# z430/keyword-spotting

Measured on AMD Instinct MI355X. Metric: 1s 16kHz clips/sec end-to-end (wav->label), higher is better.
Workload: dtype f32

## Files before the change

keyword-spotting_amd/csrc/kws_dscnn.hip:

```cpp
#include <array>
#include <utility>

#include "kws_dscnn_stages.h"

namespace kws {
namespace {

#ifndef KWS_X_DSCNN_STAMP_TID
#define KWS_X_DSCNN_STAMP_TID 0
#endif

__device__ __forceinline__ DscnnWeights weights_for_this_clip() {
#if defined(__HIP_DEVICE_COMPILE__)
    using KArg = const __attribute__((address_space(4))) DscnnWeights*;
    KArg p = (KArg)__builtin_amdgcn_kernarg_segment_ptr();
    asm volatile("" : "+s"(p));
    return *p;
#else
    return DscnnWeights{};
#endif
}

using FwdKernelFn = void (*)(DscnnWeights, const float*, int, float*, int32_t*, float*, unsigned long long*, const int*, StreamPush);
struct FwdKernelArgs {
    DscnnWeights w;
    const float* feat;
    int B;
    float* logits;
    int32_t* label;
    float* act;
    unsigned long long* stamps;
    const int* ring_hops;
    StreamPush sp;
};

__device__ __forceinline__ ScanWindows scan_windows_now() {
#if defined(__HIP_DEVICE_COMPILE__)
    using KArg = const __attribute__((address_space(4))) FwdKernelArgs*;
    KArg p = (KArg)__builtin_amdgcn_kernarg_segment_ptr();
    asm volatile("" : "+s"(p));
    return p->sp.scan;
#else
    return ScanWindows{};
#endif
}

template <bool SCAN>
__device__ __forceinline__ const float* clip_features(const float* __restrict__ feat, int clip, const ScanWindows& sw) {
    if constexpr (SCAN) {
        unsigned rec = __umulhi((unsigned)clip, sw.wpr_recip), win = (unsigned)clip - rec * sw.wpr;
        if (win >= sw.wpr) {
            win -= sw.wpr;
            ++rec;
        }
        return feat + (size_t)rec * sw.row_floats + (size_t)win * sw.win_floats;
    } else {
        return feat + (size_t)clip * (IN_T * IN_F);
    }
}

template <bool PAIR, bool SCAN = false>
__device__ __forceinline__ void stage_features_persist(float* lds, const float* __restrict__ feat, int clip, int tid,
                                                       const ScanWindows& sw = ScanWindows{}) {
    constexpr int ST = STAGE_WAVES * 64;
    constexpr int FV = (IN_T * IN_F + ST - 1) / ST;
    static_assert(2 * STAGE_WAVES == NW, "each staging wavefront zeroes the maximum slot of one other wavefront");
    const int lane = tid & 63, wv = tid >> 6;
    const float* f = clip_features<SCAN>(feat, clip, sw);
    float fv[FV];
#pragma unroll
    for (int k = 0; k < FV; ++k) {
        const int i = tid + k * ST;
        fv[k] = i < IN_T * IN_F ? f[i] : 0.f;
    }
    float* featp = lds + OFF_FEAT_P;
    for (int i = tid; i < FEAT_H * FEAT_W; i += ST) {
        const int r = i / FEAT_W - 2, c = i % FEAT_W - 2;
        if (!((unsigned)r < (unsigned)IN_T && (unsigned)c < (unsigned)IN_F)) featp[i] = 0.f;
    }
#pragma unroll
    for (int k = 0; k < FV; ++k) {
        const int i = tid + k * ST;
        if (i < IN_T * IN_F) featp[(i / IN_F + 2) * FEAT_W + (i % IN_F) + 2] = fv[k];
    }
    if constexpr (PAIR) {
        float m = 0.f;
#pragma unroll
        for (int k = 0; k < FV; ++k) m = fmaxf(m, fabsf(fv[k]));
        publish_wave_max(lds, 0, wv, lane, m);
        if (lane == 63) lds[OFF_WMAX + wv + STAGE_WAVES] = 0.f;
    }
}

__device__ __forceinline__ void pool_fc_wave(const DscnnWeights& w, const float* lds, int lane, int clip, float* __restrict__ logits,
                                             int32_t* __restrict__ label, float* __restrict__ a_pool) {
    const int C = w.num_classes;
    float4 fcw[CH / 4];
    float fcb = 0.f;
    const float4* wr = reinterpret_cast<const float4*>(w.fc_w + (lane < C ? lane : 0) * CH);
#pragma unroll
    for (int c = 0; c < CH / 4; ++c) fcw[c] = wr[c];
    if (lane < C) fcb = w.fc_b[lane];
    const float ring_b = w.pw_b[3 * CH + lane];
    constexpr float RING_N = 55.f * 11.f - 53.f * 9.f;
    float s = 0.f;
#pragma unroll
    for (int k = 0; k < NW; ++k) s += lds[OFF_POOLBUF_P + k * CH + lane];
    s = fmaf(RING_N, relu(ring_b), s) * (1.0f / (55.f * 11.f));
    if (a_pool) a_pool[lane] = s;
    float acc = fcb;
#pragma unroll
    for (int c = 0; c < CH / 4; ++c) {
        const float4 a4 = fcw[c];
        acc = fmaf(a4.x, __builtin_bit_cast(float, __builtin_amdgcn_readlane(__builtin_bit_cast(int, s), 4 * c + 0)), acc);
        acc = fmaf(a4.y, __builtin_bit_cast(float, __builtin_amdgcn_readlane(__builtin_bit_cast(int, s), 4 * c + 1)), acc);
        acc = fmaf(a4.z, __builtin_bit_cast(float, __builtin_amdgcn_readlane(__builtin_bit_cast(int, s), 4 * c + 2)), acc);
        acc = fmaf(a4.w, __builtin_bit_cast(float, __builtin_amdgcn_readlane(__builtin_bit_cast(int, s), 4 * c + 3)), acc);
    }
    if (lane < C) logits[(size_t)clip * C + lane] = acc;
    const int idx = wave_argmax_first(lane < C ? acc : -INFINITY, lane, C);
    if (label && lane == 0) label[clip] = idx;
}

template <int MODE, bool DIAG = true, bool PRECONV = false, bool STREAM = false, bool CLUSTER = false, bool PERSIST = false,
          bool SCAN = false>
__global__ __launch_bounds__(NT) void kws_dscnn_fwd_kernel(DscnnWeights w_arg, const float* __restrict__ feat, int B,
                                                           float* __restrict__ logits, int32_t* __restrict__ label,
                                                           float* __restrict__ act_arg,
                                                           unsigned long long* __restrict__ stamps_arg,
                                                           const int* __restrict__ ring_hops, StreamPush sp) {
    static_assert(!STREAM || (MODE >= 4 && !DIAG && !PRECONV), "the fused push exists for the product paths only");
    static_assert(!PERSIST || ((MODE == 4 || MODE == 5) && !PRECONV && !STREAM), "persistent workgroups: batched product paths only");
    static_assert(!SCAN || ((MODE == 4 || MODE == 5) && !DIAG && !PRECONV && !STREAM && !CLUSTER), "strided windows: batched product paths only");
    constexpr bool PAIR = MODE == 5;
    constexpr int NP = PAIR ? 2 : 3;
    BlockTables t1_pre{};
    static_assert(!CLUSTER || STREAM, "time-tile clusters exist for the streaming push only");
    float* const act = DIAG ? act_arg : nullptr;
    unsigned long long* const stamps = DIAG ? stamps_arg : nullptr;
    extern __shared__ __attribute__((aligned(16))) float lds[];
    constexpr bool MFMA = MODE != 0;
    const int tid_k = threadIdx.x;
    const int lane_k = tid_k & 63, wv_k = tid_k >> 6;

    const int cl_n = CLUSTER ? sp.cluster : 1;
    int clip = CLUSTER ? (int)blockIdx.x / cl_n : (int)blockIdx.x;
    const int cl_tile = CLUSTER ? (int)blockIdx.x - clip * cl_n : 0;
    if (clip >= B) return;
    const int j0 = Blk<4>::H * cl_tile / cl_n, j1 = Blk<4>::H * (cl_tile + 1) / cl_n;
    auto rows = [&](int lo, int hi, int H, int W) { return PosRange{(lo < 0 ? 0 : lo) * W, (hi > H ? H : hi) * W}; };
    const PosRange rg4 = rows(j0, j1, Blk<4>::H, Blk<4>::W), rg3 = rows(j0 - 2, j1, Blk<3>::H, Blk<3>::W),
                   rg2 = rows(j0 - 4, j1, Blk<2>::H, Blk<2>::W), rg1 = rows(j0 - 6, j1, Blk<1>::H, Blk<1>::W),
                   rg0 = rows(j0 - 7, j1 + 1, C1_H, C1_W);
    int n_stamp = 0;
    auto stamp = [&]() {
        if (stamps && tid_k == KWS_X_DSCNN_STAMP_TID) stamps[(size_t)clip * KWS_DSCNN_STAMPS + n_stamp] = __builtin_amdgcn_s_memtime();
        ++n_stamp;
    };

    constexpr bool SPLIT = MODE >= 4;
    BlockTables t1p{};
    uintx4 c1p[PERSIST ? 7 : 1][NP];
    int prev_clip = -1;
    float* a_prev = nullptr;
    if constexpr (PERSIST) {
        fetch_block_tables(w_arg, 1, tid_k, t1p);
        if (wv_k < STAGE_WAVES) stage_features_persist<PAIR, SCAN>(lds, feat, clip, tid_k, sp.scan);
        load_conv1_frags(w_arg, wv_k, lane_k, c1p);
        __syncthreads();
    }
    for (;;) {
    const DscnnWeights w = PERSIST ? weights_for_this_clip() : w_arg;
    int tid = tid_k;
    if constexpr (PERSIST) {
        int wv_l = __builtin_amdgcn_readfirstlane(wv_k), lane_l = lane_k;
        asm volatile("" : "+s"(wv_l), "+v"(lane_l));
        tid = (wv_l << 6) | (lane_l & 63);
    }
    const int lane = tid & 63, wv = tid >> 6;
    if constexpr (PERSIST) n_stamp = 0;
    if (stamps && tid == KWS_X_DSCNN_STAMP_TID) stamps[(size_t)clip * KWS_DSCNN_STAMPS + KWS_DSCNN_STAMPS - 2] = __builtin_amdgcn_s_memrealtime();
    stamp();

    PwOperands<MODE> wa;
    int hops_before = 0;
    int kx = 0, ky[5] = {0, 0, 0, 0, 0}, sg[5] = {0, 0, 0, 0, 0};
    if constexpr (PERSIST) {
        if constexpr (PAIR) {
            const float mxf = read_stage_max(lds, 0, 1);
            kx = pow2_exp_for(mxf);
            const float bz0 = (w.c1_abs * mxf + w.c1_bmax) * 1.001f;
            cap_units(kx, sg[0], w.k_c1, bz0);
            const float by1 = (w.dw_abs[0] * bz0 + w.dw_bmax[0]) * 1.001f;
            ky[1] = pow2_exp_for(by1);
            cap_units(ky[1], sg[1], w.k_pw[0], (w.pw_abs[0] * by1 + w.pw_bmax[0]) * 1.001f);
            store_block_tables(lds, 1, tid, t1p, pow2f(ky[1]), pow2f(sg[1]), pow2f(ky[1] - sg[0]));
            conv1_build_windows(lds, tid, pow2f(kx), OFF_FEAT_P);
            __syncthreads();
        } else {
            store_block_tables(lds, 1, tid, t1p);
        }
        stamp();
        conv1_phase_split<false, NP>(w, lds, tid, c1p, rg0, pow2f(kx), pow2f(sg[0]), OFF_FEAT_P);
        if (wv == NW - 1 && prev_clip >= 0) {
            pool_fc_wave(w, lds, lane, prev_clip, logits, label, a_prev);
            if (stamps && lane == 0) stamps[(size_t)prev_clip * KWS_DSCNN_STAMPS + 13] = __builtin_amdgcn_s_memtime();
        }
        load_afrag(w, 1, wv >= 4 ? wv - 4 : 0, lane, wa.ring[0]);
    } else if constexpr (PRECONV) {
        static_assert(!PRECONV || MODE >= 4, "the pre-convolved entry exists for the product (split) path only");
        const float* z = feat + (size_t)clip * (CH * P0);
        fetch_block_tables(w, 1, tid, t1_pre);
        float zmax = 0.f;
        for (int i = tid; i < CH * P0; i += NT) {
            const float v = z[i];
            lds[OFF_Z0 + pidx(i / P0, i % P0, P0 + 2)] = v;
            zmax = fmaxf(zmax, v);
        }
        if (tid < CH) {
            lds[OFF_Z0 + pidx(tid, P0, P0 + 2)] = 0.f;
            lds[OFF_Z0 + pidx(tid, P0 + 1, P0 + 2)] = 0.f;
        }
        if constexpr (PAIR)
            publish_wave_max(lds, 1, wv, lane, zmax);
        else
            store_block_tables(lds, 1, tid, t1_pre);
        if constexpr (Leftover<1>::HAS && (MODE == 4 || MODE == 5) && !CLUSTER)
            load_afrag(w, 1, wv >= 4 ? wv - 4 : 0, lane, wa.ring[0]);
        else
            load_block_head(w, 1, lane, wa);
        stamp();
    } else {
    float* featp = lds + OFF_FEAT;
    const float* f = clip_features<SCAN>(feat, clip, sp.scan);
    constexpr int FV = (IN_T * IN_F + NT - 1) / NT;
    float fv[FV];
    int row_new = -1;
    int head;
    if constexpr (STREAM) {
        hops_before = *sp.hops;
        const int K = (sp.p.frame_len + sp.p.frame_step - 1) / sp.p.frame_step;
        head = (((hops_before + 2 - K) % IN_T) + IN_T) % IN_T;
        const int step = sp.p.frame_step;
        const long f_start = (long)step * hops_before + step - (long)((sp.p.frame_len + step - 1) / step) * step;
        if (f_start >= 0) row_new = (int)((((f_start / step) - head) % IN_T + IN_T) % IN_T);
    } else {
        head = ring_hops ? (((*ring_hops + 1 - sp.frames_lag) % IN_T) + IN_T) % IN_T : 0;
    }
#pragma unroll
    for (int k = 0; k < FV; ++k) {
        const int i = tid + k * NT;
        fv[k] = (i < IN_T * IN_F && i / IN_F != row_new) ? f[((i / IN_F + head) % IN_T) * IN_F + i % IN_F] : 0.f;
    }
    BlockTables t1;
    fetch_block_tables(w, 1, tid, t1);
    __builtin_amdgcn_sched_barrier(0);
    float a1[SPLIT ? 1 : 50];
    uintx4 c1f[SPLIT ? 7 : 1][NP];
    if constexpr (SPLIT) {
        load_conv1_frags(w, wv, lane, c1f);
    } else if constexpr (MFMA) {
        const int half = lane >> 5, col = lane & 31, ct = wv & 1;
#pragma unroll
        for (int s = 0; s < 50; ++s) a1[s] = w.c1_w[(2 * s + half) * CH + ct * 32 + col];
        load_pointwise(w, 1, lane, wa);
    }
    __builtin_amdgcn_sched_barrier(0);
    if constexpr (PAIR) {
        float m = 0.f;
#pragma unroll
        for (int k = 0; k < FV; ++k) m = fmaxf(m, fabsf(fv[k]));
        publish_wave_max(lds, 0, wv, lane, m);
    }
    if constexpr (STREAM) {
#ifdef KWS_X_STREAM_NO_FRAME
        if (false)
#else
        if (wv == 0 && cl_tile == cl_n - 1)
#endif
            stream_frame_wave(sp.p, sp.t, sp.hop, clip, clip, false, sp.pcm_ring, sp.ring_len, const_cast<float*>(feat), hops_before,
                              reinterpret_cast<unsigned char*>(lds + OFF_Z2), lane,
                              row_new >= 0 ? featp + (row_new + 2) * FEAT_W + 2 : nullptr, sp.refine_ctr);
        for (int i = tid; i < FEAT_H * FEAT_W; i += NT) {
            const int r = i / FEAT_W - 2, c = i % FEAT_W - 2;
            if (!((unsigned)r < (unsigned)IN_T && (unsigned)c < (unsigned)IN_F)) featp[i] = 0.f;
        }
        if constexpr (!PAIR) store_block_tables(lds, 1, tid, t1);
#pragma unroll
        for (int k = 0; k < FV; ++k) {
            const int i = tid + k * NT;
            if (i < IN_T * IN_F && i / IN_F != row_new) featp[(i / IN_F + 2) * FEAT_W + (i % IN_F) + 2] = fv[k];
        }
        __syncthreads();
    } else {
    for (int i = tid; i < FEAT_H * FEAT_W; i += NT) {
        const int r = i / FEAT_W - 2, c = i % FEAT_W - 2;
        if (!((unsigned)r < (unsigned)IN_T && (unsigned)c < (unsigned)IN_F)) featp[i] = 0.f;
    }
    if constexpr (!PAIR) store_block_tables(lds, 1, tid, t1);
#pragma unroll
    for (int k = 0; k < FV; ++k) {
        const int i = tid + k * NT;
        if (i < IN_T * IN_F) featp[(i / IN_F + 2) * FEAT_W + (i % IN_F) + 2] = fv[k];
    }
    __syncthreads();
    }
    if constexpr (PAIR) {
        float mxf = read_stage_max(lds, 0, 1);
        if constexpr (STREAM) {
            if (row_new >= 0 && cl_tile == cl_n - 1)
                for (int c = 0; c < IN_F; ++c) mxf = fmaxf(mxf, fabsf(featp[(row_new + 2) * FEAT_W + 2 + c]));
        }
        kx = pow2_exp_for(mxf);
        const float bz0 = (w.c1_abs * mxf + w.c1_bmax) * 1.001f;
        cap_units(kx, sg[0], w.k_c1, bz0);
        const float by1 = (w.dw_abs[0] * bz0 + w.dw_bmax[0]) * 1.001f;
        ky[1] = pow2_exp_for(by1);
        cap_units(ky[1], sg[1], w.k_pw[0], (w.pw_abs[0] * by1 + w.pw_bmax[0]) * 1.001f);
        store_block_tables(lds, 1, tid, t1, pow2f(ky[1]), pow2f(sg[1]), pow2f(ky[1] - sg[0]));
        conv1_build_windows(lds, tid, pow2f(kx));
        __syncthreads();
    }
    stamp();

    if constexpr (SPLIT) {
        conv1_phase_split<CLUSTER, NP>(w, lds, tid, c1f, rg0, pow2f(kx), pow2f(sg[0]));
        if constexpr (Leftover<1>::HAS && (MODE == 4 || MODE == 5) && !CLUSTER)
            load_afrag(w, 1, wv >= 4 ? wv - 4 : 0, lane, wa.ring[0]);
        else
            load_block_head(w, 1, lane, wa);
    } else {
        conv1_phase<MFMA>(w, lds, tid, a1);
    }
    }
    stamp();
    __syncthreads();
    stamp();
    float* a = act ? act + (size_t)clip * KWS_ACT_FLOATS_PER_CLIP : nullptr;
    constexpr bool KSL_ON = (MODE == 4 || MODE == 5) && !CLUSTER;
    if (a) {
        const float u = PAIR ? pow2f(-sg[0]) : 1.f;
        for (int i = tid; i < CH * P0; i += NT) a[i] = lds[OFF_Z0 + pidx(i / P0, i % P0, P0 + 2)] * u;
        a += CH * P0;
    }
    PairCtx pc;
    if constexpr (PAIR && PRECONV) {
        const float mz0 = read_stage_max(lds, 1, 1);
        const float by1 = (w.dw_abs[0] * mz0 + w.dw_bmax[0]) * 1.001f;
        ky[1] = pow2_exp_for(by1);
        cap_units(ky[1], sg[1], w.k_pw[0], (w.pw_abs[0] * by1 + w.pw_bmax[0]) * 1.001f);
        store_block_tables(lds, 1, tid, t1_pre, pow2f(ky[1]), pow2f(sg[1]), pow2f(ky[1]));
        __syncthreads();
    }
    if constexpr (PAIR) {
        const float mz = read_stage_max(lds, 1, 1) * pow2f(-sg[0]);
        const float bz = (w.pw_abs[0] * ((w.dw_abs[0] * mz + w.dw_bmax[0]) * 1.001f) + w.pw_bmax[0]) * 1.001f;
        const float by = (w.dw_abs[1] * bz + w.dw_bmax[1]) * 1.001f;
        ky[2] = pow2_exp_for(by);
        cap_units(ky[2], sg[2], w.k_pw[1], (w.pw_abs[1] * by + w.pw_bmax[1]) * 1.001f);
        pc.s_dww = pow2f(ky[2] - sg[1]);
        pc.s_dwb = pow2f(ky[2]);
        pc.s_pwb = pow2f(sg[2]);
    }
    block_phase<1, MODE, CLUSTER>(w, lds, tid, wa, nullptr, rg1, pc);
    stamp();
    __syncthreads();
    if constexpr (Leftover<1>::HAS && KSL_ON) {
        leftover_combine<1, PAIR>(lds, tid);
        __syncthreads();
    }
    stamp();
    if (a) {
        const float u = PAIR ? pow2f(-sg[1]) : 1.f;
        for (int i = tid; i < CH * Blk<1>::POUT; i += NT)
            a[i] = lds[OFF_Z1 + pidx(i / Blk<1>::POUT, i % Blk<1>::POUT, Blk<1>::SOUT)] * u;
        a += CH * Blk<1>::POUT;
    }
    if constexpr (PAIR) {
        const float mz = fmaxf(read_stage_max(lds, 2, (Leftover<1>::HAS && KSL_ON) ? 2 : 1) * pow2f(-sg[1]), w.pw_bmax[0]);
        const float bz = (w.pw_abs[1] * ((w.dw_abs[1] * mz + w.dw_bmax[1]) * 1.001f) + w.pw_bmax[1]) * 1.001f;
        const float by = (w.dw_abs[2] * bz + w.dw_bmax[2]) * 1.001f;
        ky[3] = pow2_exp_for(by);
        cap_units(ky[3], sg[3], w.k_pw[2], (w.pw_abs[2] * by + w.pw_bmax[2]) * 1.001f);
        pc.s_dww = pow2f(ky[3] - sg[2]);
        pc.s_dwb = pow2f(ky[3]);
        pc.s_pwb = pow2f(sg[3]);
    }
    block_phase<2, MODE, CLUSTER>(w, lds, tid, wa, nullptr, rg2, pc);
    stamp();
    __syncthreads();
    if constexpr (Leftover<2>::HAS && KSL_ON) {
        leftover_combine<2, PAIR>(lds, tid);
        __syncthreads();
    }
    stamp();
    if (a) {
        const float u = PAIR ? pow2f(-sg[2]) : 1.f;
        for (int i = tid; i < CH * Blk<2>::POUT; i += NT)
            a[i] = lds[OFF_Z2 + pidx(i / Blk<2>::POUT, i % Blk<2>::POUT, Blk<2>::SOUT)] * u;
        a += CH * Blk<2>::POUT;
    }
    if constexpr (PAIR) {
        const float mz = fmaxf(read_stage_max(lds, 0, (Leftover<2>::HAS && KSL_ON) ? 2 : 1) * pow2f(-sg[2]), w.pw_bmax[1]);
        const float bz = (w.pw_abs[2] * ((w.dw_abs[2] * mz + w.dw_bmax[2]) * 1.001f) + w.pw_bmax[2]) * 1.001f;
        const float by = (w.dw_abs[3] * bz + w.dw_bmax[3]) * 1.001f;
        ky[4] = pow2_exp_for(by);
        cap_units(ky[4], sg[4], w.k_pw[3], (w.pw_abs[3] * by + w.pw_bmax[3]) * 1.001f);
        pc.s_dww = pow2f(ky[4] - sg[3]);
        pc.s_dwb = pow2f(ky[4]);
        pc.s_pwb = pow2f(sg[4]);
    }
    block_phase<3, MODE, CLUSTER>(w, lds, tid, wa, nullptr, rg3, pc);
    stamp();
    __syncthreads();
    stamp();
    if (a) {
        const float u = PAIR ? pow2f(-sg[3]) : 1.f;
        for (int i = tid; i < CH * Blk<3>::POUT; i += NT)
            a[i] = lds[OFF_Z3 + pidx(i / Blk<3>::POUT, i % Blk<3>::POUT, Blk<3>::SOUT)] * u;
        a += CH * Blk<3>::POUT;
    }
    if constexpr (PAIR) {
        pc.inv_out = pow2f(-sg[4]);
    }
    block_phase<4, MODE, CLUSTER>(w, lds, tid, wa, a ? a + CH : nullptr, rg4, pc,
                                  PERSIST ? OFF_POOLBUF_P : OFF_POOLBUF);
    stamp();
    if constexpr (PERSIST) {
        const int next = clip + (int)gridDim.x;
        __builtin_amdgcn_sched_barrier(0);
        const ScanWindows sw_next = SCAN ? scan_windows_now() : ScanWindows{};
        if (wv < STAGE_WAVES && next < B) stage_features_persist<PAIR, SCAN>(lds, feat, next, tid, sw_next);
        stamp();
        load_conv1_frags(w, wv, lane, c1p);
        __syncthreads();
        stamp();
        if (stamps && tid == KWS_X_DSCNN_STAMP_TID) stamps[(size_t)clip * KWS_DSCNN_STAMPS + KWS_DSCNN_STAMPS - 1] = __builtin_amdgcn_s_memrealtime();
        prev_clip = clip;
        a_prev = a;
        clip = next;
        if (clip >= B) break;
        continue;
    }
    const int C = w.num_classes;
    float4 fcw[CH / 4];
    float fcb = 0.f, ring_b = 0.f;
    if (wv == 0 && lane < C) {
        const float4* wr = reinterpret_cast<const float4*>(w.fc_w + lane * CH);
#pragma unroll
        for (int c = 0; c < CH / 4; ++c) fcw[c] = wr[c];
        fcb = w.fc_b[lane];
    }
    if (tid < CH) ring_b = w.pw_b[3 * CH + tid];
    __syncthreads();
    stamp();

    float* pooled = lds + OFF_POOLED;
    constexpr float RING_N = 55.f * 11.f - 53.f * 9.f;
    bool run_fc = true;
    if constexpr (CLUSTER) {
        float* part = sp.cl_part + ((size_t)clip * cl_n + cl_tile) * CH;
        if (tid < CH) {
            float s = 0.f;
#pragma unroll
            for (int k = 0; k < NW; ++k) s += lds[OFF_POOLBUF + k * CH + tid];
            __hip_atomic_store(part + tid, s, __ATOMIC_RELAXED, __HIP_MEMORY_SCOPE_AGENT);
        }
        asm volatile("s_waitcnt vmcnt(0)" ::: "memory");
        __syncthreads();
        int* last_flag = reinterpret_cast<int*>(lds + OFF_POOLED + CH);
        if (tid == 0) {
            const int arrived = atomicAdd(&sp.cl_count[clip], 1);
            *last_flag = arrived == cl_n - 1;
            if (arrived == cl_n - 1) sp.cl_count[clip] = 0;
        }
        __syncthreads();
        run_fc = *last_flag != 0;
        if (run_fc) {
            if (tid < CH) {
                float s = 0.f;
                for (int t = 0; t < cl_n; ++t)
                    s += __hip_atomic_load(sp.cl_part + ((size_t)clip * cl_n + t) * CH + tid, __ATOMIC_RELAXED, __HIP_MEMORY_SCOPE_AGENT);
                pooled[tid] = fmaf(RING_N, relu(ring_b), s) * (1.0f / (55.f * 11.f));
            }
        }
        __syncthreads();
    } else {
    if (tid < CH) {
        float s = 0.f;
#pragma unroll
        for (int k = 0; k < NW; ++k) s += lds[OFF_POOLBUF + k * CH + tid];
        s = fmaf(RING_N, relu(ring_b), s) * (1.0f / (55.f * 11.f));
        pooled[tid] = s;
        if (a) a[tid] = s;
    }
    __syncthreads();
    }

    if (run_fc && wv == 0) {
        float v = -INFINITY;
        if (lane < C) {
            float acc = fcb;
            const float4* pl = reinterpret_cast<const float4*>(pooled);
#pragma unroll
            for (int c = 0; c < CH / 4; ++c) {
                const float4 a4 = fcw[c], p4 = pl[c];
                acc = fmaf(a4.x, p4.x, acc);
                acc = fmaf(a4.y, p4.y, acc);
                acc = fmaf(a4.z, p4.z, acc);
                acc = fmaf(a4.w, p4.w, acc);
            }
            logits[(size_t)clip * C + lane] = acc;
            if constexpr (STREAM) {
                if (sp.h_logits) __hip_atomic_store(sp.h_logits + (size_t)clip * C + lane, acc, __ATOMIC_RELAXED, __HIP_MEMORY_SCOPE_SYSTEM);
            }
            v = acc;
        }
        const int idx = wave_argmax_first(v, lane, C);
        if (label && lane == 0) label[clip] = idx;
        if constexpr (STREAM) {
            if (sp.h_label && lane == 0) __hip_atomic_store(sp.h_label + clip, idx, __ATOMIC_RELAXED, __HIP_MEMORY_SCOPE_SYSTEM);
        }
    }
    if constexpr (STREAM) {
        int finishers = (int)gridDim.x;
        if constexpr (CLUSTER) finishers /= cl_n;
        if (sp.h_flag) asm volatile("s_waitcnt vmcnt(0)" ::: "memory");
        if (run_fc && tid == 0 && atomicAdd(&sp.hops[1], 1) == finishers - 1) {
            sp.hops[1] = 0;
            sp.hops[0] = hops_before + 1;
            if (sp.h_flag) __hip_atomic_store(sp.h_flag, hops_before + 1, __ATOMIC_RELAXED, __HIP_MEMORY_SCOPE_SYSTEM);
        }
    }
    stamp();
    if (stamps && tid == KWS_X_DSCNN_STAMP_TID) stamps[(size_t)clip * KWS_DSCNN_STAMPS + KWS_DSCNN_STAMPS - 1] = __builtin_amdgcn_s_memrealtime();
    break;
    }
    if constexpr (PERSIST) {
        if (wv_k == NW - 1) {
            pool_fc_wave(w_arg, lds, lane_k, prev_clip, logits, label, a_prev);
            if (stamps && lane_k == 0) stamps[(size_t)prev_clip * KWS_DSCNN_STAMPS + 13] = __builtin_amdgcn_s_memtime();
        }
    }
}

enum : unsigned { F_DIAG = 1, F_PRECONV = 2, F_STREAM = 4, F_CLUSTER = 8, F_PERSIST = 16, F_SCAN = 32 };
struct FwdVariant {
    int mode;
    unsigned flags;
    bool diag, preconv, stream, cluster, persist, scan;
    constexpr FwdVariant(int m, unsigned f)
        : mode(m), flags(f), diag(f & F_DIAG), preconv(f & F_PRECONV), stream(f & F_STREAM), cluster(f & F_CLUSTER), persist(f & F_PERSIST), scan(f & F_SCAN) {}
};
constexpr FwdVariant kFwdVariants[] = {
    {0, F_DIAG},
    {1, F_DIAG},
    {2, F_DIAG},
    {3, F_DIAG},
    {4, F_DIAG},
    {6, F_DIAG},
    {4, 0},
    {4, F_PRECONV},
    {4, F_STREAM},
    {4, F_STREAM | F_CLUSTER},
    {5, F_DIAG},
    {5, 0},
    {5, F_PRECONV},
    {5, F_STREAM},
    {5, F_STREAM | F_CLUSTER},
    {4, F_DIAG | F_PERSIST},
    {4, F_PERSIST},
    {5, F_DIAG | F_PERSIST},
    {5, F_PERSIST},
    {4, F_SCAN},
    {4, F_PERSIST | F_SCAN},
    {5, F_SCAN},
    {5, F_PERSIST | F_SCAN},
};
constexpr size_t N_FWD_VARIANTS = sizeof(kFwdVariants) / sizeof(kFwdVariants[0]);

template <size_t I>
constexpr auto kFwdKernel = &kws_dscnn_fwd_kernel<kFwdVariants[I].mode, kFwdVariants[I].diag, kFwdVariants[I].preconv, kFwdVariants[I].stream,
                                                  kFwdVariants[I].cluster, kFwdVariants[I].persist, kFwdVariants[I].scan>;
template <size_t... I>
constexpr std::array<FwdKernelFn, sizeof...(I)> fwd_kernel_table(std::index_sequence<I...>) {
    return {{kFwdKernel<I>...}};
}
constexpr auto kFwdKernels = fwd_kernel_table(std::make_index_sequence<N_FWD_VARIANTS>{});

static_assert(std::is_same_v<decltype(kFwdKernel<0>), const FwdKernelFn>,
              "kws_dscnn_fwd_kernel's parameters and FwdKernelArgs / FwdKernelFn must change together");

hipError_t launch_variant(int mode, unsigned flags, int grid, hipStream_t s, const DscnnWeights& w, const float* d_feat, int B, float* d_logits,
                          int32_t* d_label, float* d_act, unsigned long long* d_stamps, const int* d_ring_hops, const StreamPush& sp) {
    for (size_t i = 0; i < N_FWD_VARIANTS; ++i) {
        if (kFwdVariants[i].mode != mode || kFwdVariants[i].flags != flags) continue;
        hipLaunchKernelGGL(kFwdKernels[i], dim3(grid), dim3(NT), LDS_FLOATS * sizeof(float), s, w, d_feat, B, d_logits, d_label, d_act, d_stamps,
                           d_ring_hops, sp);
        return hipGetLastError();
    }
    return hipErrorInvalidValue;
}

}

hipError_t dscnn_init_device() {
    for (FwdKernelFn k : kFwdKernels) {
        hipError_t e = hipFuncSetAttribute(reinterpret_cast<const void*>(k), hipFuncAttributeMaxDynamicSharedMemorySize, LDS_FLOATS * (int)sizeof(float));
        if (e != hipSuccess) return e;
    }
    return hipSuccess;
}

hipError_t launch_dscnn_stream(hipStream_t s, const DscnnWeights& w, const StreamPush& sp, float* d_feat_ring, int n_streams,
                               float* d_logits, int32_t* d_label, bool pair) {
    static_assert(sizeof(float) * (size_t)(LDS_FLOATS - OFF_Z2) >= 16 * 1024 + STREAM_F64_BYTES, "room for the one-frame front end's tables and scratch");
    const bool tiles = sp.cluster > 1;
    return launch_variant(pair ? 5 : 4, tiles ? F_STREAM | F_CLUSTER : F_STREAM, tiles ? n_streams * sp.cluster : n_streams, s, w, d_feat_ring,
                          n_streams, d_logits, d_label, nullptr, nullptr, nullptr, sp);
}

hipError_t launch_dscnn(hipStream_t s, const DscnnWeights& w, const float* d_feat, int B, float* d_logits,
                        int32_t* d_label, float* d_act, int mode, unsigned long long* d_stamps, const int* d_ring_hops,
// ... 24 lines not shown
```

keyword-spotting_amd/csrc/kws_dscnn_stages.h:

```cpp
#pragma once
#include <type_traits>

#include "kws_dscnn_geom.h"
#include "kws_mfcc_dev.h"
#include "kws_split_mfma.h"

namespace kws {
namespace {

template <bool TO_MFMA = false>
__device__ __forceinline__ float stencil3x3(float w0, float w1, float w2, float w3, float w4, float w5, float w6,
                                            float w7, float w8, float b, float up, float mid, float dn, float mask_l,
                                            float mask_r) {
    float c, to_right, to_left;
    asm("v_mul_f32 %1, %3, %13\n\t"
        "v_mul_f32 %2, %5, %13\n\t"
        "v_fma_f32 %0, %4, %13, %12\n\t"
        "v_fmac_f32 %1, %6, %14\n\t"
        "v_fmac_f32 %2, %8, %14\n\t"
        "v_fmac_f32 %0, %7, %14\n\t"
        "v_fmac_f32 %1, %9, %15\n\t"
        "v_fmac_f32 %2, %11, %15\n\t"
        "v_fmac_f32 %0, %10, %15\n\t"
        "v_fmac_f32_dpp %0, %1, %16 wave_shr:1 row_mask:0xf bank_mask:0xf bound_ctrl:1\n\t"
// ... 313 lines not shown
template <bool DUAL>
__device__ __forceinline__ void conv1_unit_pairwin(const DscnnWeights& w, const float* lds, float* z0, int ptile, int ct, int lane,
                                                   const uintx4 (&c1f)[7][2], int p_lo, int p_hi, float sig0, float& mx) {
    const int half = lane >> 5, col = lane & 31;
    const int pos = p_lo + ptile * 32 + col;
    const int posc = pos < p_hi ? pos : p_hi - 1;
    const int oh = posc / C1_W, ow = posc % C1_W;
    const int wi = (2 * oh + 5 * half) * 3 + ow;
    const uintx4* w8 = reinterpret_cast<const uintx4*>(lds + OFF_C1W8) + wi;
    const uint32_t* p2 = reinterpret_cast<const uint32_t*>(lds + OFF_C1P2) + wi;
    const floatx16 zero = {0, 0, 0, 0, 0, 0, 0, 0, 0, 0, 0, 0, 0, 0, 0, 0};
    floatx16 acc = zero, acc2 = zero, occ = zero, occ2 = zero;
    const uintx4* osrc = reinterpret_cast<const uintx4*>(w.c1_pair) + (size_t)(ct ^ 1) * (7 * 2 * 64) + lane;
    uintx4 of[DUAL ? 7 : 1][2];
    if (DUAL) {
#pragma unroll
        for (int kb = 0; kb < 7; ++kb) {
            of[kb][0] = osrc[(kb * 2 + 0) * 64];
            of[kb][1] = osrc[(kb * 2 + 1) * 64];
        }
    }
    float4 cb[4], ob[DUAL ? 4 : 1];
#pragma unroll
    for (int q = 0; q < 4; ++q) {
        cb[q] = *reinterpret_cast<const float4*>(w.c1_b + ct * 32 + 8 * q + 4 * half);
        if (DUAL) ob[DUAL ? q : 0] = *reinterpret_cast<const float4*>(w.c1_b + (ct ^ 1) * 32 + 8 * q + 4 * half);
    }
    uintx4 bq[3][2];
    auto b_load = [&](int kb, uintx4 (&d)[2]) {
        if (kb < 5) {
            d[0] = w8[kb * 3];
            d[1] = w8[kb * 3 + C1W_ROWS * 3];
        } else if (kb == 5) {
#pragma unroll
            for (int i = 0; i < 4; ++i) {
                d[0][i] = p2[i * 3];
                d[1][i] = p2[i * 3 + C1W_ROWS * 3];
            }
        } else {
            d[0] = uintx4{p2[4 * 3], 0u, 0u, 0u};
            d[1] = uintx4{p2[4 * 3 + C1W_ROWS * 3], 0u, 0u, 0u};
        }
    };
    b_load(0, bq[0]);
    b_load(1, bq[1]);
#pragma unroll
    for (int kb = 0; kb < 7; ++kb) {
        if (kb + 2 < 7) b_load(kb + 2, bq[(kb + 2) % 3]);
        const uintx4 &bh = bq[kb % 3][0], &bl = bq[kb % 3][1];
        acc2 = mfma_f16(c1f[kb][0], bl, acc2);
        if (DUAL) occ2 = mfma_f16(of[DUAL ? kb : 0][0], bl, occ2);
        acc = mfma_f16(c1f[kb][1], bh, acc);
        if (DUAL) occ = mfma_f16(of[DUAL ? kb : 0][1], bh, occ);
        acc2 = mfma_f16(c1f[kb][0], bh, acc2);
        if (DUAL) occ2 = mfma_f16(of[DUAL ? kb : 0][0], bh, occ2);
    }
    acc += acc2;
    occ += occ2;
    if (pos < p_hi) {
#pragma unroll
        for (int r = 0; r < 16; r += 2) {
            const int co = ct * 32 + row_of(r, half);
            const float4 b4 = cb[r >> 2];
            const float b0 = (r & 2) ? b4.z : b4.x, b1 = (r & 2) ? b4.w : b4.y;
            const float v0 = relu(fmaf(b0, sig0, acc[r])), v1 = relu(fmaf(b1, sig0, acc[r + 1]));
            *reinterpret_cast<float2*>(z0 + pidx(co, pos, P0 + 2)) = make_float2(v0, v1);
            mx = fmaxf(mx, fmaxf(v0, v1));
            if (DUAL) {
                const int oo = (ct ^ 1) * 32 + row_of(r, half);
                const float4 o4 = ob[DUAL ? (r >> 2) : 0];
                const float c0 = (r & 2) ? o4.z : o4.x, c1 = (r & 2) ? o4.w : o4.y;
                const float u0 = relu(fmaf(c0, sig0, occ[r])), u1 = relu(fmaf(c1, sig0, occ[r + 1]));
                *reinterpret_cast<float2*>(z0 + pidx(oo, pos, P0 + 2)) = make_float2(u0, u1);
                mx = fmaxf(mx, fmaxf(u0, u1));
            }
        }
    }
}

struct PosRange {
    int lo, hi;
};

template <bool RANGED, int NP>
__device__ __forceinline__ void conv1_phase_split(const DscnnWeights& w, float* lds, int tid, const uintx4 (&c1f)[7][NP],
                                                  PosRange rg, float sx = 1.f, float sig0 = 1.f, int off_feat = OFF_FEAT) {
    static_assert(P0 > 4 * 32 && P0 <= 5 * 32 && NW >= 6, "conv1 work split: four dual tiles + one tile in two halves");
    const float* featp = lds + off_feat;
    float* z0 = lds + OFF_Z0;
    const int lane = tid & 63, wv = tid >> 6;
    float mx = 0.f;
    if constexpr (NP == 2) {
        if constexpr (RANGED) {
            const int n_pt = (rg.hi - rg.lo + 31) / 32;
            for (int u = wv; u < 2 * n_pt; u += NW) conv1_unit_pairwin<false>(w, lds, z0, u >> 1, u & 1, lane, c1f, rg.lo, rg.hi, sig0, mx);
        } else if (wv < 4)
            conv1_unit_pairwin<true>(w, lds, z0, wv, wv & 1, lane, c1f, 0, P0, sig0, mx);
        else if (wv < 6)
            conv1_unit_pairwin<false>(w, lds, z0, 4, wv & 1, lane, c1f, 0, P0, sig0, mx);
    } else if constexpr (RANGED) {
        const int n_pt = (rg.hi - rg.lo + 31) / 32;
        for (int u = wv; u < 2 * n_pt; u += NW) conv1_unit_split<false, NP>(w, featp, z0, u >> 1, u & 1, lane, c1f, rg.lo, rg.hi, sx, sig0, mx);
    } else if (wv < 4)
        conv1_unit_split<true, NP>(w, featp, z0, wv, wv & 1, lane, c1f, 0, P0, sx, sig0, mx);
    else if (wv < 6)
        conv1_unit_split<false, NP>(w, featp, z0, 4, wv & 1, lane, c1f, 0, P0, sx, sig0, mx);
    if constexpr (NP == 2) publish_wave_max(lds, 1, wv, lane, mx);
    if (tid < CH) {
        z0[pidx(tid, P0, P0 + 2)] = 0.f;
        z0[pidx(tid, P0 + 1, P0 + 2)] = 0.f;
    }
}

template <int N, int NP>
__device__ __forceinline__ void leftover_partial_unit(float* lds, int lane, int M, const uintx4 (&af)[2][NP]) {
    using G = Blk<N>;
    using L = Leftover<N>;
    const int half = lane >> 5, col = lane & 31;
    const float* dwtab = lds + OFF_DWTAB + G::BUF * 768;
    const float4* dwt4 = reinterpret_cast<const float4*>(dwtab) + half * 24;
    const int pos = L::P0T - 1 + col;
    const bool valid = col >= 1 && col <= TW && pos < G::POUT;
    const int posc = pos < G::POUT ? pos : G::POUT - 1;
    const int h = posc / G::W, x = posc % G::W;
    const float mask_l = x > 0 ? 1.f : 0.f, mask_r = x < G::W - 1 ? 1.f : 0.f;
    int ta[3];
#pragma unroll
    for (int dh = -1; dh <= 1; ++dh) {
        const int o = G::RING ? 1 : 0;
        const int hh = h + dh - o, xx = x - o;
        const bool inside = (unsigned)hh < (unsigned)G::HI && (unsigned)xx < (unsigned)G::WI;
        const bool in_map = (unsigned)(h + dh) < (unsigned)G::H;
        const int a = inside ? hh * G::WI + xx : ((G::RING && in_map) ? G::PIN : G::PIN + 1);
        ta[dh + 1] = G::OFF_IN + pidx(half * 8, a, G::SIN);
    }
    float y[8];
#pragma unroll
    for (int j = 0; j < 8; j += 2) {
        const int cs = 16 * M + j;
        const int o = cs * G::SIN;
        const float2 up = *reinterpret_cast<const float2*>(lds + ta[0] + o);
        const float2 mid = *reinterpret_cast<const float2*>(lds + ta[1] + o);
        const float2 dn = *reinterpret_cast<const float2*>(lds + ta[2] + o);
        DwPair wp;
#pragma unroll
        for (int i = 0; i < 5; ++i) wp.l[i] = dwt4[(cs >> 1) * 6 + i];
        y[j] = stencil3x3_of_pair<false, 0>(wp, up.x, mid.x, dn.x, mask_l, mask_r);
        y[j + 1] = stencil3x3_of_pair<false, 1>(wp, up.y, mid.y, dn.y, mask_l, mask_r);
    }
    floatx16 acc0 = {0, 0, 0, 0, 0, 0, 0, 0, 0, 0, 0, 0, 0, 0, 0, 0}, acc1 = acc0;
    if constexpr (NP == 2) {
        uintx4 bh, bl;
        split_pair8_scaled(y, bh, bl);
        acc0 = mfma_f16(af[0][0], bl, acc0);
        acc1 = mfma_f16(af[1][0], bl, acc1);
        acc0 = mfma_f16(af[0][1], bh, acc0);
        acc1 = mfma_f16(af[1][1], bh, acc1);
        acc0 = mfma_f16(af[0][0], bh, acc0);
        acc1 = mfma_f16(af[1][0], bh, acc1);
    } else {
        uintx4 bh, bm, bl;
        split3(y, bh, bm, bl);
#pragma unroll
        for (int q = 0; q < 6; ++q) {
            const int pa = q == 0 ? 2 : (q == 2 || q == 3) ? 1 : 0;
            const uintx4& b = (q == 0 || q == 3 || q == 5) ? bh : (q == 1 ? bl : bm);
            acc0 = mfma_bf16(af[0][pa], b, acc0);
            acc1 = mfma_bf16(af[1][pa], b, acc1);
        }
    }
    float* part = lds + L::OFF_PART + M * (CH * L::NP);
    if (valid) {
#pragma unroll
        for (int r = 0; r < 16; ++r) {
            part[row_of(r, half) * L::NP + (col - 1)] = acc0[r];
            part[(32 + row_of(r, half)) * L::NP + (col - 1)] = acc1[r];
        }
    }
}

template <int N, bool PAIR = false>
// ... 328 lines not shown
                    "v_add_f32_dpp %9, %9, %9 row_shr:1 row_mask:0xf bank_mask:0xf bound_ctrl:1\n\t"
                    "v_add_f32_dpp %10, %10, %10 row_shr:1 row_mask:0xf bank_mask:0xf bound_ctrl:1\n\t"
                    "v_add_f32_dpp %11, %11, %11 row_shr:1 row_mask:0xf bank_mask:0xf bound_ctrl:1\n\t"
                    "v_add_f32_dpp %12, %12, %12 row_shr:1 row_mask:0xf bank_mask:0xf bound_ctrl:1\n\t"
                    "v_add_f32_dpp %13, %13, %13 row_shr:1 row_mask:0xf bank_mask:0xf bound_ctrl:1\n\t"
                    "v_add_f32_dpp %14, %14, %14 row_shr:1 row_mask:0xf bank_mask:0xf bound_ctrl:1\n\t"
                    "v_add_f32_dpp %15, %15, %15 row_shr:1 row_mask:0xf bank_mask:0xf bound_ctrl:1\n\t"
                    "v_add_f32_dpp %0, %0, %0 row_shr:2 row_mask:0xf bank_mask:0xf bound_ctrl:1\n\t"
                    "v_add_f32_dpp %1, %1, %1 row_shr:2 row_mask:0xf bank_mask:0xf bound_ctrl:1\n\t"
                    "v_add_f32_dpp %2, %2, %2 row_shr:2 row_mask:0xf bank_mask:0xf bound_ctrl:1\n\t"
                    "v_add_f32_dpp %3, %3, %3 row_shr:2 row_mask:0xf bank_mask:0xf bound_ctrl:1\n\t"
                    "v_add_f32_dpp %4, %4, %4 row_shr:2 row_mask:0xf bank_mask:0xf bound_ctrl:1\n\t"
                    "v_add_f32_dpp %5, %5, %5 row_shr:2 row_mask:0xf bank_mask:0xf bound_ctrl:1\n\t"
                    "v_add_f32_dpp %6, %6, %6 row_shr:2 row_mask:0xf bank_mask:0xf bound_ctrl:1\n\t"
                    "v_add_f32_dpp %7, %7, %7 row_shr:2 row_mask:0xf bank_mask:0xf bound_ctrl:1\n\t"
                    "v_add_f32_dpp %8, %8, %8 row_shr:2 row_mask:0xf bank_mask:0xf bound_ctrl:1\n\t"
                    "v_add_f32_dpp %9, %9, %9 row_shr:2 row_mask:0xf bank_mask:0xf bound_ctrl:1\n\t"
                    "v_add_f32_dpp %10, %10, %10 row_shr:2 row_mask:0xf bank_mask:0xf bound_ctrl:1\n\t"
                    "v_add_f32_dpp %11, %11, %11 row_shr:2 row_mask:0xf bank_mask:0xf bound_ctrl:1\n\t"
                    "v_add_f32_dpp %12, %12, %12 row_shr:2 row_mask:0xf bank_mask:0xf bound_ctrl:1\n\t"
                    "v_add_f32_dpp %13, %13, %13 row_shr:2 row_mask:0xf bank_mask:0xf bound_ctrl:1\n\t"
                    "v_add_f32_dpp %14, %14, %14 row_shr:2 row_mask:0xf bank_mask:0xf bound_ctrl:1\n\t"
                    "v_add_f32_dpp %15, %15, %15 row_shr:2 row_mask:0xf bank_mask:0xf bound_ctrl:1\n\t"
                    "v_add_f32_dpp %0, %0, %0 row_shr:4 row_mask:0xf bank_mask:0xf bound_ctrl:1\n\t"
                    "v_add_f32_dpp %1, %1, %1 row_shr:4 row_mask:0xf bank_mask:0xf bound_ctrl:1\n\t"
                    "v_add_f32_dpp %2, %2, %2 row_shr:4 row_mask:0xf bank_mask:0xf bound_ctrl:1\n\t"
                    "v_add_f32_dpp %3, %3, %3 row_shr:4 row_mask:0xf bank_mask:0xf bound_ctrl:1\n\t"
                    "v_add_f32_dpp %4, %4, %4 row_shr:4 row_mask:0xf bank_mask:0xf bound_ctrl:1\n\t"
                    "v_add_f32_dpp %5, %5, %5 row_shr:4 row_mask:0xf bank_mask:0xf bound_ctrl:1\n\t"
                    "v_add_f32_dpp %6, %6, %6 row_shr:4 row_mask:0xf bank_mask:0xf bound_ctrl:1\n\t"
                    "v_add_f32_dpp %7, %7, %7 row_shr:4 row_mask:0xf bank_mask:0xf bound_ctrl:1\n\t"
                    "v_add_f32_dpp %8, %8, %8 row_shr:4 row_mask:0xf bank_mask:0xf bound_ctrl:1\n\t"
                    "v_add_f32_dpp %9, %9, %9 row_shr:4 row_mask:0xf bank_mask:0xf bound_ctrl:1\n\t"
                    "v_add_f32_dpp %10, %10, %10 row_shr:4 row_mask:0xf bank_mask:0xf bound_ctrl:1\n\t"
                    "v_add_f32_dpp %11, %11, %11 row_shr:4 row_mask:0xf bank_mask:0xf bound_ctrl:1\n\t"
                    "v_add_f32_dpp %12, %12, %12 row_shr:4 row_mask:0xf bank_mask:0xf bound_ctrl:1\n\t"
                    "v_add_f32_dpp %13, %13, %13 row_shr:4 row_mask:0xf bank_mask:0xf bound_ctrl:1\n\t"
                    "v_add_f32_dpp %14, %14, %14 row_shr:4 row_mask:0xf bank_mask:0xf bound_ctrl:1\n\t"
                    "v_add_f32_dpp %15, %15, %15 row_shr:4 row_mask:0xf bank_mask:0xf bound_ctrl:1\n\t"
                    "v_add_f32_dpp %0, %0, %0 row_shr:8 row_mask:0xf bank_mask:0xf bound_ctrl:1\n\t"
                    "v_add_f32_dpp %1, %1, %1 row_shr:8 row_mask:0xf bank_mask:0xf bound_ctrl:1\n\t"
                    "v_add_f32_dpp %2, %2, %2 row_shr:8 row_mask:0xf bank_mask:0xf bound_ctrl:1\n\t"
                    "v_add_f32_dpp %3, %3, %3 row_shr:8 row_mask:0xf bank_mask:0xf bound_ctrl:1\n\t"
                    "v_add_f32_dpp %4, %4, %4 row_shr:8 row_mask:0xf bank_mask:0xf bound_ctrl:1\n\t"
                    "v_add_f32_dpp %5, %5, %5 row_shr:8 row_mask:0xf bank_mask:0xf bound_ctrl:1\n\t"
                    "v_add_f32_dpp %6, %6, %6 row_shr:8 row_mask:0xf bank_mask:0xf bound_ctrl:1\n\t"
                    "v_add_f32_dpp %7, %7, %7 row_shr:8 row_mask:0xf bank_mask:0xf bound_ctrl:1\n\t"
                    "v_add_f32_dpp %8, %8, %8 row_shr:8 row_mask:0xf bank_mask:0xf bound_ctrl:1\n\t"
                    "v_add_f32_dpp %9, %9, %9 row_shr:8 row_mask:0xf bank_mask:0xf bound_ctrl:1\n\t"
                    "v_add_f32_dpp %10, %10, %10 row_shr:8 row_mask:0xf bank_mask:0xf bound_ctrl:1\n\t"
                    "v_add_f32_dpp %11, %11, %11 row_shr:8 row_mask:0xf bank_mask:0xf bound_ctrl:1\n\t"
                    "v_add_f32_dpp %12, %12, %12 row_shr:8 row_mask:0xf bank_mask:0xf bound_ctrl:1\n\t"
                    "v_add_f32_dpp %13, %13, %13 row_shr:8 row_mask:0xf bank_mask:0xf bound_ctrl:1\n\t"
                    "v_add_f32_dpp %14, %14, %14 row_shr:8 row_mask:0xf bank_mask:0xf bound_ctrl:1\n\t"
                    "v_add_f32_dpp %15, %15, %15 row_shr:8 row_mask:0xf bank_mask:0xf bound_ctrl:1\n\t"
                    "v_add_f32_dpp %0, %0, %0 row_bcast:15 row_mask:0xa bank_mask:0xf\n\t"
                    "v_add_f32_dpp %1, %1, %1 row_bcast:15 row_mask:0xa bank_mask:0xf\n\t"
                    "v_add_f32_dpp %2, %2, %2 row_bcast:15 row_mask:0xa bank_mask:0xf\n\t"
                    "v_add_f32_dpp %3, %3, %3 row_bcast:15 row_mask:0xa bank_mask:0xf\n\t"
                    "v_add_f32_dpp %4, %4, %4 row_bcast:15 row_mask:0xa bank_mask:0xf\n\t"
                    "v_add_f32_dpp %5, %5, %5 row_bcast:15 row_mask:0xa bank_mask:0xf\n\t"
                    "v_add_f32_dpp %6, %6, %6 row_bcast:15 row_mask:0xa bank_mask:0xf\n\t"
                    "v_add_f32_dpp %7, %7, %7 row_bcast:15 row_mask:0xa bank_mask:0xf\n\t"
                    "v_add_f32_dpp %8, %8, %8 row_bcast:15 row_mask:0xa bank_mask:0xf\n\t"
                    "v_add_f32_dpp %9, %9, %9 row_bcast:15 row_mask:0xa bank_mask:0xf\n\t"
                    "v_add_f32_dpp %10, %10, %10 row_bcast:15 row_mask:0xa bank_mask:0xf\n\t"
                    "v_add_f32_dpp %11, %11, %11 row_bcast:15 row_mask:0xa bank_mask:0xf\n\t"
                    "v_add_f32_dpp %12, %12, %12 row_bcast:15 row_mask:0xa bank_mask:0xf\n\t"
                    "v_add_f32_dpp %13, %13, %13 row_bcast:15 row_mask:0xa bank_mask:0xf\n\t"
                    "v_add_f32_dpp %14, %14, %14 row_bcast:15 row_mask:0xa bank_mask:0xf\n\t"
                    "v_add_f32_dpp %15, %15, %15 row_bcast:15 row_mask:0xa bank_mask:0xf"
                    : "+v"(q[0]), "+v"(q[1]), "+v"(q[2]), "+v"(q[3]), "+v"(q[4]), "+v"(q[5]), "+v"(q[6]), "+v"(q[7]), "+v"(q[8]), "+v"(q[9]), "+v"(q[10]), "+v"(q[11]), "+v"(q[12]), "+v"(q[13]), "+v"(q[14]), "+v"(q[15]));
            }
            if (col == 31) {
#pragma unroll
                for (int k = 0; k < 32; ++k) poolbuf[wv * CH + (k >> 4) * 32 + row_of(k & 15, half)] = psum[k >> 4][k & 15] * pc.inv_out;
            }
        }
    }
    (void)bias4;
}

template <int NP>
__device__ __forceinline__ void load_conv1_frags(const DscnnWeights& w, int wv, int lane, uintx4 (&c1f)[7][NP]) {
    const uintx4* src = reinterpret_cast<const uintx4*>(NP == 2 ? w.c1_pair : w.c1_split) + (size_t)(wv & 1) * (7 * NP * 64) + lane;
#pragma unroll
    for (int kb = 0; kb < 7; ++kb)
#pragma unroll
        for (int p = 0; p < NP; ++p) c1f[kb][p] = src[(kb * NP + p) * 64];
}

__device__ __forceinline__ int wave_argmax_first(float v, int lane, int C) {
    float m = v;
    m = fmaxf(m, __builtin_bit_cast(float, __builtin_amdgcn_update_dpp(__builtin_bit_cast(int, m), __builtin_bit_cast(int, m), 0x111, 0xf, 0xf, false)));
    m = fmaxf(m, __builtin_bit_cast(float, __builtin_amdgcn_update_dpp(__builtin_bit_cast(int, m), __builtin_bit_cast(int, m), 0x112, 0xf, 0xf, false)));
    m = fmaxf(m, __builtin_bit_cast(float, __builtin_amdgcn_update_dpp(__builtin_bit_cast(int, m), __builtin_bit_cast(int, m), 0x114, 0xf, 0xf, false)));
    m = fmaxf(m, __builtin_bit_cast(float, __builtin_amdgcn_update_dpp(__builtin_bit_cast(int, m), __builtin_bit_cast(int, m), 0x118, 0xf, 0xf, false)));
    m = fmaxf(m, __builtin_bit_cast(float, __builtin_amdgcn_update_dpp(__builtin_bit_cast(int, m), __builtin_bit_cast(int, m), 0x142, 0xa, 0xf, false)));
    m = fmaxf(m, __builtin_bit_cast(float, __builtin_amdgcn_update_dpp(__builtin_bit_cast(int, m), __builtin_bit_cast(int, m), 0x143, 0xc, 0xf, false)));
    const float vmax = __builtin_bit_cast(float, __builtin_amdgcn_readlane(__builtin_bit_cast(int, m), 63));
    const unsigned long long holders = __ballot(lane < C && v == vmax);
    return holders ? __ffsll(holders) - 1 : 0;
}

}
}
```

Measured before the change: 7.062 million.

## Rebalance conv1 work across eight waves and defer previous clip's FC past block 1

In the persistent pair path, the conv1 work split changes. Previously four dual-tile waves plus two half-tile waves did the work and two waves idled. Now ten single units are spread over all eight wavefronts, with each wave's channel tile chosen by wv>>2. The pooled-FC epilogue for the previous clip is also split up. The pool sum is read early, before conv1 overwrites the buffers, and the FC matmul and argmax now run after the first block phase instead of right after conv1. The aim is to shorten the conv1 critical path and hide the FC wave's work behind block 1, at the cost of extra registers and a possibly uneven load on waves 0 and 5.

```diff
diff --git a/keyword-spotting_amd/csrc/kws_dscnn.hip b/keyword-spotting_amd/csrc/kws_dscnn.hip
--- a/keyword-spotting_amd/csrc/kws_dscnn.hip
+++ b/keyword-spotting_amd/csrc/kws_dscnn.hip
@@ -92,26 +92,35 @@
     }
 }
 
-__device__ __forceinline__ void pool_fc_wave(const DscnnWeights& w, const float* lds, int lane, int clip, float* __restrict__ logits,
-                                             int32_t* __restrict__ label, float* __restrict__ a_pool) {
+constexpr int FC_WAVE = NW - 1;
+struct FcOperands {
+    float4 fcw[CH / 4];
+    float fcb, ring_b;
+};
+__device__ __forceinline__ float pool_take(const float* lds, int lane) {
+    float s = 0.f;
+#pragma unroll
+    for (int k = 0; k < NW; ++k) s += lds[OFF_POOLBUF_P + k * CH + lane];
+    return s;
+}
+__device__ __forceinline__ void fc_request(const DscnnWeights& w, int lane, FcOperands& o) {
     const int C = w.num_classes;
-    float4 fcw[CH / 4];
-    float fcb = 0.f;
     const float4* wr = reinterpret_cast<const float4*>(w.fc_w + (lane < C ? lane : 0) * CH);
 #pragma unroll
-    for (int c = 0; c < CH / 4; ++c) fcw[c] = wr[c];
-    if (lane < C) fcb = w.fc_b[lane];
-    const float ring_b = w.pw_b[3 * CH + lane];
+    for (int c = 0; c < CH / 4; ++c) o.fcw[c] = wr[c];
+    o.fcb = lane < C ? w.fc_b[lane] : 0.f;
+    o.ring_b = w.pw_b[3 * CH + lane];
+}
+__device__ __forceinline__ void fc_finish(const DscnnWeights& w, const FcOperands& o, float s, int lane, int clip,
+                                          float* __restrict__ logits, int32_t* __restrict__ label, float* __restrict__ a_pool) {
+    const int C = w.num_classes;
     constexpr float RING_N = 55.f * 11.f - 53.f * 9.f;
-    float s = 0.f;
-#pragma unroll
-    for (int k = 0; k < NW; ++k) s += lds[OFF_POOLBUF_P + k * CH + lane];
-    s = fmaf(RING_N, relu(ring_b), s) * (1.0f / (55.f * 11.f));
+    s = fmaf(RING_N, relu(o.ring_b), s) * (1.0f / (55.f * 11.f));
     if (a_pool) a_pool[lane] = s;
-    float acc = fcb;
+    float acc = o.fcb;
 #pragma unroll
     for (int c = 0; c < CH / 4; ++c) {
-        const float4 a4 = fcw[c];
+        const float4 a4 = o.fcw[c];
         acc = fmaf(a4.x, __builtin_bit_cast(float, __builtin_amdgcn_readlane(__builtin_bit_cast(int, s), 4 * c + 0)), acc);
         acc = fmaf(a4.y, __builtin_bit_cast(float, __builtin_amdgcn_readlane(__builtin_bit_cast(int, s), 4 * c + 1)), acc);
         acc = fmaf(a4.z, __builtin_bit_cast(float, __builtin_amdgcn_readlane(__builtin_bit_cast(int, s), 4 * c + 2)), acc);
@@ -159,6 +168,7 @@
     };
 
     constexpr bool SPLIT = MODE >= 4;
+    constexpr int C1SPLIT = (PERSIST && PAIR) ? KWS_DSCNN_CONV1_SPLIT : 0;
     BlockTables t1p{};
     uintx4 c1p[PERSIST ? 7 : 1][NP];
     int prev_clip = -1;
@@ -166,7 +176,7 @@
     if constexpr (PERSIST) {
         fetch_block_tables(w_arg, 1, tid_k, t1p);
         if (wv_k < STAGE_WAVES) stage_features_persist<PAIR, SCAN>(lds, feat, clip, tid_k, sp.scan);
-        load_conv1_frags(w_arg, wv_k, lane_k, c1p);
+        load_conv1_frags(w_arg, conv1_ct<C1SPLIT>(wv_k), lane_k, c1p);
         __syncthreads();
     }
     for (;;) {
@@ -185,7 +195,9 @@
     PwOperands<MODE> wa;
     int hops_before = 0;
     int kx = 0, ky[5] = {0, 0, 0, 0, 0}, sg[5] = {0, 0, 0, 0, 0};
+    float pool_s = 0.f;
     if constexpr (PERSIST) {
+        if (wv == FC_WAVE && prev_clip >= 0) pool_s = pool_take(lds, lane);
         if constexpr (PAIR) {
             const float mxf = read_stage_max(lds, 0, 1);
             kx = pow2_exp_for(mxf);
@@ -201,11 +213,7 @@
             store_block_tables(lds, 1, tid, t1p);
         }
         stamp();
-        conv1_phase_split<false, NP>(w, lds, tid, c1p, rg0, pow2f(kx), pow2f(sg[0]), OFF_FEAT_P);
-        if (wv == NW - 1 && prev_clip >= 0) {
-            pool_fc_wave(w, lds, lane, prev_clip, logits, label, a_prev);
-            if (stamps && lane == 0) stamps[(size_t)prev_clip * KWS_DSCNN_STAMPS + 13] = __builtin_amdgcn_s_memtime();
-        }
+        conv1_phase_split<false, NP, C1SPLIT>(w, lds, tid, c1p, rg0, pow2f(kx), pow2f(sg[0]), OFF_FEAT_P);
         load_afrag(w, 1, wv >= 4 ? wv - 4 : 0, lane, wa.ring[0]);
     } else if constexpr (PRECONV) {
         static_assert(!PRECONV || MODE >= 4, "the pre-convolved entry exists for the product (split) path only");
@@ -258,7 +266,7 @@
     float a1[SPLIT ? 1 : 50];
     uintx4 c1f[SPLIT ? 7 : 1][NP];
     if constexpr (SPLIT) {
-        load_conv1_frags(w, wv, lane, c1f);
+        load_conv1_frags(w, wv & 1, lane, c1f);
     } else if constexpr (MFMA) {
         const int half = lane >> 5, col = lane & 31, ct = wv & 1;
 #pragma unroll
@@ -362,7 +370,23 @@
         pc.s_dwb = pow2f(ky[2]);
         pc.s_pwb = pow2f(sg[2]);
     }
+    auto fc_prev = [&]() {
+        if constexpr (PERSIST) {
+            if (wv == FC_WAVE && prev_clip >= 0) {
+                FcOperands fco;
+                fc_request(w, lane, fco);
+                fc_finish(w, fco, pool_s, lane, prev_clip, logits, label, a_prev);
+                if (stamps && lane == 0) stamps[(size_t)prev_clip * KWS_DSCNN_STAMPS + 13] = __builtin_amdgcn_s_memtime();
+            }
+        }
+    };
+#ifdef KWS_X_DSCNN_FC_BEFORE_QUARTER
+    fc_prev();
+#endif
     block_phase<1, MODE, CLUSTER>(w, lds, tid, wa, nullptr, rg1, pc);
+#ifndef KWS_X_DSCNN_FC_BEFORE_QUARTER
+    fc_prev();
+#endif
     stamp();
     __syncthreads();
     if constexpr (Leftover<1>::HAS && KSL_ON) {
@@ -432,7 +456,7 @@
         const ScanWindows sw_next = SCAN ? scan_windows_now() : ScanWindows{};
         if (wv < STAGE_WAVES && next < B) stage_features_persist<PAIR, SCAN>(lds, feat, next, tid, sw_next);
         stamp();
-        load_conv1_frags(w, wv, lane, c1p);
+        load_conv1_frags(w, conv1_ct<C1SPLIT>(wv), lane, c1p);
         __syncthreads();
         stamp();
         if (stamps && tid == KWS_X_DSCNN_STAMP_TID) stamps[(size_t)clip * KWS_DSCNN_STAMPS + KWS_DSCNN_STAMPS - 1] = __builtin_amdgcn_s_memrealtime();
@@ -537,8 +561,10 @@
     break;
     }
     if constexpr (PERSIST) {
-        if (wv_k == NW - 1) {
-            pool_fc_wave(w_arg, lds, lane_k, prev_clip, logits, label, a_prev);
+        if (wv_k == FC_WAVE) {
+            FcOperands fcl;
+            fc_request(w_arg, lane_k, fcl);
+            fc_finish(w_arg, fcl, pool_take(lds, lane_k), lane_k, prev_clip, logits, label, a_prev);
             if (stamps && lane_k == 0) stamps[(size_t)prev_clip * KWS_DSCNN_STAMPS + 13] = __builtin_amdgcn_s_memtime();
         }
     }
diff --git a/keyword-spotting_amd/csrc/kws_dscnn_stages.h b/keyword-spotting_amd/csrc/kws_dscnn_stages.h
--- a/keyword-spotting_amd/csrc/kws_dscnn_stages.h
+++ b/keyword-spotting_amd/csrc/kws_dscnn_stages.h
@@ -419,10 +419,19 @@
     int lo, hi;
 };
 
-template <bool RANGED, int NP>
+#ifndef KWS_DSCNN_CONV1_SPLIT
+#define KWS_DSCNN_CONV1_SPLIT 1
+#endif
+template <int SPLIT>
+__device__ __forceinline__ constexpr int conv1_ct(int wv) {
+    return SPLIT == 1 ? wv >> 2 : wv & 1;
+}
+template <bool RANGED, int NP, int SPLIT = 0>
 __device__ __forceinline__ void conv1_phase_split(const DscnnWeights& w, float* lds, int tid, const uintx4 (&c1f)[7][NP],
                                                   PosRange rg, float sx = 1.f, float sig0 = 1.f, int off_feat = OFF_FEAT) {
+    static_assert(SPLIT == 0 || NW == 8, "ten single units, or the fifth tile on wavefronts 6 and 7: eight wavefronts");
     static_assert(P0 > 4 * 32 && P0 <= 5 * 32 && NW >= 6, "conv1 work split: four dual tiles + one tile in two halves");
+    static_assert(SPLIT == 0 || (NP == 2 && !RANGED), "the other splits read the pre-split windows of a whole map");
     const float* featp = lds + off_feat;
     float* z0 = lds + OFF_Z0;
     const int lane = tid & 63, wv = tid >> 6;
@@ -431,9 +440,17 @@
         if constexpr (RANGED) {
             const int n_pt = (rg.hi - rg.lo + 31) / 32;
             for (int u = wv; u < 2 * n_pt; u += NW) conv1_unit_pairwin<false>(w, lds, z0, u >> 1, u & 1, lane, c1f, rg.lo, rg.hi, sig0, mx);
+        } else if constexpr (SPLIT == 1) {
+            const int n_units = (wv == 0 || wv == 5) ? 2 : 1;
+#pragma unroll 1
+            for (int u = 0; u < n_units; ++u) conv1_unit_pairwin<false>(w, lds, z0, u ? 4 : wv & 3, wv >> 2, lane, c1f, 0, P0, sig0, mx);
+        } else if constexpr (SPLIT == 3) {
+            const int n_units = wv < 2 ? 2 : 1;
+#pragma unroll 1
+            for (int u = 0; u < n_units; ++u) conv1_unit_pairwin<false>(w, lds, z0, u ? 4 : wv >> 1, wv & 1, lane, c1f, 0, P0, sig0, mx);
         } else if (wv < 4)
             conv1_unit_pairwin<true>(w, lds, z0, wv, wv & 1, lane, c1f, 0, P0, sig0, mx);
-        else if (wv < 6)
+        else if (SPLIT == 2 ? wv >= 6 : wv < 6)
             conv1_unit_pairwin<false>(w, lds, z0, 4, wv & 1, lane, c1f, 0, P0, sig0, mx);
     } else if constexpr (RANGED) {
         const int n_pt = (rg.hi - rg.lo + 31) / 32;
@@ -928,8 +945,8 @@
 }
 
 template <int NP>
-__device__ __forceinline__ void load_conv1_frags(const DscnnWeights& w, int wv, int lane, uintx4 (&c1f)[7][NP]) {
-    const uintx4* src = reinterpret_cast<const uintx4*>(NP == 2 ? w.c1_pair : w.c1_split) + (size_t)(wv & 1) * (7 * NP * 64) + lane;
+__device__ __forceinline__ void load_conv1_frags(const DscnnWeights& w, int ct, int lane, uintx4 (&c1f)[7][NP]) {
+    const uintx4* src = reinterpret_cast<const uintx4*>(NP == 2 ? w.c1_pair : w.c1_split) + (size_t)ct * (7 * NP * 64) + lane;
 #pragma unroll
     for (int kb = 0; kb < 7; ++kb)
 #pragma unroll
```

New measurement: 7.116 million (median of 6 runs). Within noise of the previous version (+0.8%).
